# TalShor/SciLMM

Measured on AMD Instinct MI355X. Metric: REML factorize+solve nnz(L)/s (simulated pedigree, fp64), higher is better.
Workload: dtype f64

## Files before the change

scilmm_amd/csrc/dev.h:

```cpp
#pragma once
#include <hip/hip_runtime.h>

#include <algorithm>
#include <cstdlib>
#include <optional>
#include <string>
#include <type_traits>
#include <vector>

#include "../../include/scilmm_hip.h"
#include "plan_types.h"
#include "handles.h"

namespace scilmm {

struct Tuning {
  int reserve_cus = 0;
  int side_streams = 2;
  bool no_mfma = false;
  bool trsm_lite = true;
  std::optional<bool> dense;
  std::optional<bool> outside;
  bool outside_merge = true;
  std::optional<int> outside_chunks;
  bool outside_prio = false;
  std::optional<double> cell_limit;
  bool no_lookahead = false;
  int look_depth = 2;
  bool host_cells = false;
  bool no_splitk = false;
  int64_t target_items = 1024;
  int64_t min_item = 24;
  int64_t max_item = 96;
  std::optional<int64_t> dense_items;
  int64_t dense_fill = 256;
  std::optional<bool> dense_taper;
  std::optional<int> dist_group;
  bool dist_nosplit = false;
  int chain_cap = 2048;
  int chain_wide = 12;
  bool no_chain = false;
  int64_t push_slice = 512;
  bool shadow = true;
  int chain_wide_t = 256;
  int chain_full_t = 768;
  bool sinv_generic = false;
};

inline Tuning read_tuning() {
  Tuning t;
  const char* gate = getenv("SCILMM_TUNING");
  if (!(gate && gate[0] == '1')) return t;
  auto env = [](const char* name) { return getenv(name); };
  auto is1 = [&](const char* name) { const char* e = env(name); return e && e[0] == '1'; };
  auto not0 = [&](const char* name) { const char* e = env(name); return !(e && e[0] == '0'); };
  const char* e;
  if ((e = env("SCILMM_RESERVE_CUS"))) t.reserve_cus = atoi(e);
  if ((e = env("SCILMM_SIDE_STREAMS"))) t.side_streams = atoi(e);
  t.no_mfma = is1("SCILMM_NO_MFMA");
  t.trsm_lite = not0("SCILMM_TRSM_LITE");
  if ((e = env("SCILMM_DENSE"))) t.dense = e[0] != '0';
  if ((e = env("SCILMM_OUTSIDE"))) t.outside = e[0] != '0';
  t.outside_merge = not0("SCILMM_OUTSIDE_MERGE");
  if ((e = env("SCILMM_OUTSIDE_CHUNKS"))) t.outside_chunks = atoi(e);
  t.outside_prio = is1("SCILMM_OUTSIDE_PRIO");
  if ((e = env("SCILMM_CELL_LIMIT"))) t.cell_limit = atof(e);
  t.no_lookahead = is1("SCILMM_NO_LOOKAHEAD");
  if ((e = env("SCILMM_LOOK_DEPTH"))) t.look_depth = std::max(1, atoi(e));
  t.host_cells = is1("SCILMM_HOST_CELLS");
  t.no_splitk = is1("SCILMM_NO_SPLITK");
  if ((e = env("SCILMM_TARGET_ITEMS"))) t.target_items = atoll(e);
  if ((e = env("SCILMM_MIN_ITEM"))) t.min_item = atoll(e);
  if ((e = env("SCILMM_MAX_ITEM"))) t.max_item = atoll(e);
  if ((e = env("SCILMM_DENSE_ITEMS"))) t.dense_items = atoll(e);
  if ((e = env("SCILMM_DENSE_FILL"))) t.dense_fill = atoll(e);
  if ((e = env("SCILMM_DENSE_TAPER"))) t.dense_taper = e[0] == '1';
  if ((e = env("SCILMM_DIST_GROUP"))) t.dist_group = atoi(e);
  t.dist_nosplit = is1("SCILMM_DIST_NOSPLIT");
  if ((e = env("SCILMM_CHAIN_CAP"))) t.chain_cap = atoi(e);
  if ((e = env("SCILMM_CHAIN_WIDE"))) t.chain_wide = atoi(e);
  t.no_chain = is1("SCILMM_NO_CHAIN");
  if ((e = env("SCILMM_PUSH_SLICE"))) t.push_slice = atoll(e);
  t.shadow = not0("SCILMM_SHADOW");
  if ((e = env("SCILMM_CHAIN_WIDE_T"))) t.chain_wide_t = atoi(e);
  if ((e = env("SCILMM_CHAIN_FULL_T"))) t.chain_full_t = atoi(e);
  t.sinv_generic = is1("SCILMM_SINV_GENERIC");
  return t;
}

inline bool verbose() { return getenv("SCILMM_VERBOSE") != nullptr; }

struct Dev {
  int device = 0;
  hipStream_t stream = nullptr;
  Tuning tune;
  int prio_lo = 0, prio_hi = 0;
  DevSym v{};
  std::vector<void*> allocs;
  int32_t* d_level_tiles = nullptr;
  int32_t* d_level_fronts = nullptr;
  int32_t* d_level_pairs = nullptr;
  int32_t* d_all_fronts = nullptr;
  std::vector<double*> vals;
  std::vector<uint8_t> have_vals;
  double* W = nullptr;
  double* X = nullptr;
  double* IO = nullptr;
  size_t io_cap = 0;
  double* partial = nullptr;
  int64_t nwaves_quad = 0;
  double* d_out = nullptr;
  bool use_mfma = true;
  bool trsm_lite = true;
  hipEvent_t ev[8];
  scilmm_timing timing{};
  bool quad_pending = false;
  bool attrs_set = false;
  ComboDesc* d_combos = nullptr;
// ... 49 lines not shown
  std::vector<hipEvent_t> batch_ev;
  std::vector<hipEvent_t> bpev;
  std::vector<int32_t> last_own_level;
  hipStream_t bstream = nullptr;
  hipStream_t comm = nullptr;
  std::vector<hipEvent_t> done_ev;
  double* ACC = nullptr;
  int32_t* d_col_front = nullptr;
  int64_t* d_yoff = nullptr;
  double* d_ybuf = nullptr;
  int32_t* d_sinv_pre_tiles = nullptr;
  std::vector<int64_t> sinv_pre_ptr;
  std::vector<int32_t> sinv_tail_front;
  int32_t* d_sinv_tail_fronts = nullptr;
  SinvWork* d_sinv_work = nullptr;
  std::vector<int64_t> sinv_work_ptr;
  bool work_external = false;
  bool outside_on = false;
  int32_t tail_level = 0;
  std::vector<uint8_t> outside_desc;
  OutsideWork* d_owork = nullptr;
  int32_t* d_grp_next = nullptr;
  int32_t* d_grp_t0 = nullptr;
  int64_t n_owork = 0;
  int32_t* d_tail_front = nullptr;
  uint8_t* d_keep_front = nullptr;
  hipStream_t outside_st = nullptr;
  std::vector<int64_t> ochunk_ptr;
  std::vector<hipEvent_t> out_evs;
  std::vector<int32_t> out_wait_chunk;
  bool dense_on = false;
  int front_bits = 64;
  double* d_zeros = nullptr;
  DenseWork* d_dwork_e = nullptr;
  DenseWork* d_dwork_l = nullptr;
  std::vector<int64_t> dwork_e_ptr, dwork_l_ptr;
  std::vector<int64_t> dwork_l_mid;
  int64_t n_late_split = 0;
  int look_depth = 2;
  int rhs_pending = -1;
  int32_t chain_T = 0, chain_l0 = 0;
  int32_t* d_chain = nullptr;
  int32_t* d_colmap = nullptr;
  int32_t* d_cf_ptr = nullptr;
  ChainPair* d_cf = nullptr;
  int32_t* d_cb_ptr = nullptr;
  ChainPair* d_cb = nullptr;
  int64_t* d_cg_ptr = nullptr;
  int32_t* d_cg_pairs = nullptr;
  int64_t chain_groups = 0;
  int32_t* d_cg_slot = nullptr;
  int32_t* d_fold = nullptr;
  int64_t n_fold = 0;
  double* d_push_partial = nullptr;
  int32_t* d_chain_flags = nullptr;
  int32_t* d_chain_err = nullptr;
  int32_t* h_chain_err = nullptr;
  int32_t chain_epoch = 0;
  std::vector<hipEvent_t> pev;
  bool det = false;
  PullPlan pull{};
  int32_t* d_pull_level_segs = nullptr;
  int32_t* d_pull_fold = nullptr;
  double* d_pull_partial = nullptr;
  uint8_t* d_chain_mask = nullptr;
  const int64_t* d_pat_rowptr = nullptr;
// ... 57 lines not shown
```

scilmm_amd/csrc/engine.hip:

```cpp
#include <hip/hip_runtime.h>

#include <algorithm>
#include <atomic>
#include <chrono>
#include <functional>
#include <thread>
#include <cmath>
#include <cstdio>
#include <cstdlib>
#include <cstring>
#include <string>
#include <vector>

#include "../../include/scilmm_hip.h"
#include <hipcub/hipcub.hpp>

#include "kernels.hip.h"
#include "dev.h"
#include "host_threads.h"

using namespace scilmm;

namespace {

// ... 105 lines not shown
  int32_t tail_front(int32_t l) const { return dist ? D->tail_of_level[l] : -1; }
  bool has_early(int32_t l) const {
    return D->early_ptr[l + 1] > D->early_ptr[l] || D->cellset[0].level_ptr[l + 1] > D->cellset[0].level_ptr[l] ||
           D->dwork_e_ptr[l + 1] > D->dwork_e_ptr[l];
  }
  bool deferred(int32_t le) const { return D->outside_on && le >= D->tail_level; }
  int mark(int32_t l, ProfEvent e, hipStream_t stream) {
    if (prof) HIPCHK(hipEventRecord(D->pev[(size_t)PEV_PER_LEVEL * l + e], stream));
    return SCILMM_OK;
  }

  int prepare_shadow() {
    const bool want = D->front_bits == 32 && D->dense_on && read_tuning().shadow;
    if (want && !fac->L32) {
      fac->base32 = S.sn_loff[S.dense_first];
      const size_t cnt32 = (size_t)(D->nL_local - fac->base32) + 16384;
      if (hipMalloc((void**)&fac->L32, sizeof(float) * cnt32) != hipSuccess) {
        (void)hipGetLastError();
        fac->L32 = nullptr;
      } else {
        HIPCHK(hipMemsetAsync(fac->L32, 0, sizeof(float) * cnt32, st));
      }
    } else if (!want && fac->L32) {
      HIPCHK(hipStreamSynchronize(st));
      (void)hipFree(fac->L32);
      fac->L32 = nullptr;
    }
    return SCILMM_OK;
  }

  int assemble(const double* sigma2) {
    HIPCHK(hipEventRecord(D->ev[0], st));
    HIPCHK(hipMemsetAsync(fac->L, 0, sizeof(double) * (size_t)std::max<int64_t>(D->nL_local, 1), st));
    int32_t big = 0x7fffffff;
    HIPCHK(hipMemcpyAsync(fac->status, &big, sizeof(int32_t), hipMemcpyHostToDevice, st));
    ValPtrs gen{}, dia{};
    for (int k = 0; k < S.K; ++k) {
      ValPtrs& t = S.is_diag[k] ? dia : gen;
      if (t.count >= 8) {
        sym->err = "more than 8 matrices of one kind";
        return SCILMM_ERR_ARG;
      }
      t.v[t.count] = D->vals[k];
      t.s2[t.count] = sigma2[k];
      t.count++;
    }
    if (S.nnz_pattern > 0) {
      int blocks = (int)std::min<int64_t>((S.nnz_pattern + 255) / 256, 256 * 16);
      hipLaunchKernelGGL(k_assemble, dim3(blocks), dim3(256), 0, st, S.nnz_pattern, D->v.asm_dst, gen, fac->L);
      launches++;
    }
    if (dia.count > 0 && S.n > 0) {
      hipLaunchKernelGGL(k_add_diag, dim3((S.n + 255) / 256), dim3(256), 0, st, S.n, D->v.diag_dst, dia, fac->L);
      launches++;
    }
    HIPCHK(hipEventRecord(D->ev[1], st));
    HIPCHK(hipEventRecord(D->ev_asm, st));
    HIPCHK(hipStreamWaitEvent(D->side, D->ev_asm, 0));
    HIPCHK(hipStreamWaitEvent(D->side2, D->ev_asm, 0));
    if (D->side3) HIPCHK(hipStreamWaitEvent(D->side3, D->ev_asm, 0));
    if (D->outside_st) HIPCHK(hipStreamWaitEvent(D->outside_st, D->ev_asm, 0));
    if (dist) {
      HIPCHK(hipStreamWaitEvent(D->bstream, D->ev_asm, 0));
      HIPCHK(hipStreamWaitEvent(D->comm, D->ev_asm, 0));
    }
    return SCILMM_OK;
  }

  int prepare_profiling() {
    D->n_late_split = 0;
    if (prof && D->pev.size() < (size_t)PEV_PER_LEVEL * S.nlevels) {
      size_t old = D->pev.size();
      D->pev.resize((size_t)PEV_PER_LEVEL * S.nlevels, nullptr);
      for (size_t i = old; i < D->pev.size(); ++i) HIPCHK(hipEventCreate(&D->pev[i]));
    }
    if (prof && dist && D->bpev.size() < 2 * D->batch_ev.size()) {
      size_t old = D->bpev.size();
      D->bpev.resize(2 * D->batch_ev.size(), nullptr);
      for (size_t i = old; i < D->bpev.size(); ++i) HIPCHK(hipEventCreate(&D->bpev[i]));
    }
    return SCILMM_OK;
  }

  int early(int32_t l) {
    const int64_t e0 = D->early_ptr[l], e1 = D->early_ptr[l + 1];
    if (!has_early(l)) return SCILMM_OK;
    const int sidx = D->serial_early ? 0 : l % D->nside;
    hipStream_t sd = sidx == 0 ? D->side : (sidx == 1 ? D->side2 : D->side3);
    double* scratch = D->scratch + (size_t)sidx * half;
    if (l >= D->look_depth + 1) HIPCHK(hipStreamWaitEvent(sd, D->lev_ev[2 * (l - D->look_depth - 1)], 0));
    if (D->outside_on && l >= D->tail_level && D->out_wait_chunk[(size_t)l] >= 0)
      HIPCHK(hipStreamWaitEvent(sd, D->out_evs[(size_t)D->out_wait_chunk[(size_t)l]], 0));
    TRY(mark(l, PEV_EARLY_BEGIN, sd));
    update(sd, D->d_work_early + e0, e1 - e0, scratch);
    TRY(mark(l, PEV_DENSE_E_BEGIN, sd));
    dense(sd, D->d_dwork_e + D->dwork_e_ptr[l], D->dwork_e_ptr[l + 1] - D->dwork_e_ptr[l], scratch);
    TRY(mark(l, PEV_DENSE_E_END, sd));
    TRY(mark(l, PEV_EARLY_END, sd));
    reduce(sd, D->d_red_tiles_e + D->red_ptr_e[l], D->red_ptr_e[l + 1] - D->red_ptr_e[l], D->d_tile_pslot_e, D->d_tile_pnseg_e, scratch);
    TRY(cells(sd, 0, l));
    HIPCHK(hipEventRecord(D->lev_ev[2 * l + 1], sd));
    return SCILMM_OK;
  }

  int late_updates(int32_t l) {
    double* sh = late_scratch();
    if (D->outside_on && l >= D->tail_level && D->out_wait_chunk[(size_t)l] >= 0 &&
        (l == D->tail_level || D->out_wait_chunk[(size_t)l] != D->out_wait_chunk[(size_t)l - 1]))
      HIPCHK(hipStreamWaitEvent(st, D->out_evs[(size_t)D->out_wait_chunk[(size_t)l]], 0));
    const int32_t tf = tail_front(l), Wg = D->dist_Wg;
    const int32_t jj = tf >= 0 ? tf - D->dist_first : -1, grp = tf >= 0 ? jj / Wg : -1;
    const bool own_tail = tf >= 0 && D->keep_front[tf];
    const bool split_late = own_tail && D->dwork_l_mid[(size_t)l] < D->dwork_l_ptr[l + 1];
    if (has_early(l)) HIPCHK(hipStreamWaitEvent(st, D->lev_ev[2 * l + 1], 0));
    if (own_tail) {
      if (grp >= 2) HIPCHK(hipStreamWaitEvent(st, D->batch_ev[grp - 2], 0));
      const int32_t q_end = split_late ? jj - 1 : jj;
      for (int32_t q = std::max(0, (grp - 1) * Wg); q < q_end; ++q) HIPCHK(hipStreamWaitEvent(st, D->lev_ev[2 * S.sn_level[D->dist_first + q]], 0));
    }
    TRY(mark(l, PEV_LATE_BEGIN, st));
    update(st, D->d_work + D->work_ptr[l], D->work_ptr[l + 1] - D->work_ptr[l], sh);
    TRY(mark(l, PEV_DENSE_L_BEGIN, st));
    dense(st, D->d_dwork_l + D->dwork_l_ptr[l], (split_late ? D->dwork_l_mid[(size_t)l] : D->dwork_l_ptr[l + 1]) - D->dwork_l_ptr[l], sh);
    TRY(mark(l, PEV_DENSE_L_END, st));
    if (split_late) {
      HIPCHK(hipStreamWaitEvent(st, D->lev_ev[2 * S.sn_level[D->dist_first + jj - 1]], 0));
      TRY(mark(l, PEV_DENSE_N_BEGIN, st));
      dense(st, D->d_dwork_l + D->dwork_l_mid[(size_t)l], D->dwork_l_ptr[l + 1] - D->dwork_l_mid[(size_t)l], sh);
      TRY(mark(l, PEV_DENSE_N_END, st));
      D->n_late_split++;
    }
    return mark(l, PEV_LATE_END, st);
  }

  int factor_panel(int32_t l) {
    const int64_t t0 = D->lv_tile_ptr[l], t1 = D->lv_tile_ptr[l + 1];
    const int32_t f0 = D->lv_ptr[l], f1 = D->lv_ptr[l + 1];
    const double* sh = late_scratch();
    TRY(cells(st, 1, l));
    TRY(mark(l, PEV_CELLS_END, st));
    if (f1 > f0) {
      const size_t sm_potrf = sizeof(double) * (size_t)((NB / 2) * (NB + 1) + NJB * 16 * 17 + 32);
      hipLaunchKernelGGL(k_potrf, dim3((unsigned)(f1 - f0)), dim3(256), sm_potrf, st, D->v, D->d_level_fronts + f0, fac->L,
                         fac->invD, fac->logd, fac->status, (const int32_t*)D->d_tile_pslot, (const int32_t*)D->d_tile_pnseg, sh);
      launches++;
    }
    TRY(mark(l, PEV_POTRF_END, st));
    trsm(st, D->d_level_tiles + t0, t1 - t0, sh);
    if (fac->L32) {
      for (int32_t q = f0; q < f1; ++q) {
        const int32_t fr = D->lv_fronts[(size_t)q];
        if (fr < S.dense_first || !D->keep_front[fr]) continue;
        shadow(st, fr, S.sn_loff[fr + 1] - S.sn_loff[fr]);
      }
    }
    return mark(l, PEV_LEVEL_END, st);
  }

  void shadow(hipStream_t stream, int32_t fr, int64_t cnt) {
    hipLaunchKernelGGL(k_shadow, dim3((unsigned)std::min<int64_t>((cnt + 255) / 256, 8192)), dim3(256), 0, stream,
                       (const double*)(fac->L + D->loff[fr]), fac->L32 + (D->loff[fr] - fac->base32), cnt);
// ... 6 lines not shown
    HIPCHK(hipEventRecord(D->done_ev[l], st));
    HIPCHK(hipStreamWaitEvent(D->comm, D->done_ev[l], 0));
    if (!D->keep_front[tf]) {
      const int32_t gd = (jj - D->dist_G) / D->dist_Wg;
      if (jj >= D->dist_G) {
        HIPCHK(hipStreamWaitEvent(D->comm, D->batch_ev[gd], 0));
        for (int32_t q = std::min<int32_t>(gd + 1, (int32_t)D->last_own_level.size() - 1); q >= 0; --q)
          if (D->last_own_level[q] >= 0) {
            HIPCHK(hipStreamWaitEvent(D->comm, D->done_ev[D->last_own_level[q]], 0));
            break;
          }
      }
    }
    const int64_t pm = S.sn_rowptr[tf + 1] - S.sn_rowptr[tf], pw = S.sn_start[tf + 1] - S.sn_start[tf];
    int rcm = sym->comm_fn(sym->comm_ctx, 0, 0, D->loff[tf], pm * pw, root);
    if (rcm == 0) rcm = sym->comm_fn(sym->comm_ctx, 0, 1, S.inv_off[tf], pw * pw, root);
    if (rcm == 0) rcm = sym->comm_fn(sym->comm_ctx, 0, 2, tf, 1, root);
    if (rcm != 0) {
      sym->err = "multi-GPU: the communication callback failed";
      return SCILMM_ERR_DEVICE;
    }
    if (fac->L32 && !D->keep_front[tf]) shadow(D->comm, tf, pm * pw);
    HIPCHK(hipEventRecord(D->lev_ev[2 * l], D->comm));
    last_tail_level = l;
    return SCILMM_OK;
  }

  int batch(int32_t grp) {
    hipStream_t bs = D->bstream;
    const int32_t q_end = std::min((grp + 1) * D->dist_Wg, S.nsuper - D->dist_first);
    for (int32_t q = grp * D->dist_Wg; q < q_end; ++q) HIPCHK(hipStreamWaitEvent(bs, D->lev_ev[2 * S.sn_level[D->dist_first + q]], 0));
    if (D->outside_on) HIPCHK(hipStreamWaitEvent(bs, D->out_evs.back(), 0));
    if (prof) HIPCHK(hipEventRecord(D->bpev[2 * (size_t)grp], bs));
    dense(bs, D->d_dwork_b + D->dbatch_ptr[grp], D->dbatch_ptr[grp + 1] - D->dbatch_ptr[grp], nullptr);
    if (prof) HIPCHK(hipEventRecord(D->bpev[2 * (size_t)grp + 1], bs));
    HIPCHK(hipEventRecord(D->batch_ev[grp], bs));
    return SCILMM_OK;
  }

  int outside_and_deferred_early(int32_t l) {
    HIPCHK(hipStreamWaitEvent(D->outside_st, D->lev_ev[2 * l], 0));
    for (size_t og = 0; og + 1 < D->ochunk_ptr.size(); ++og) {
      outside(D->outside_st, (const OutsideWork*)D->d_owork + D->ochunk_ptr[og], D->ochunk_ptr[og + 1] - D->ochunk_ptr[og]);
      HIPCHK(hipGetLastError());
      HIPCHK(hipEventRecord(D->out_evs[og], D->outside_st));
    }
    for (int32_t le = std::max(D->tail_level, 1); le <= l + D->look_depth && le < S.nlevels; ++le) TRY(early(le));
    return SCILMM_OK;
  }

  int exchange_status() {
    if (last_tail_level >= 0) HIPCHK(hipStreamWaitEvent(st, D->lev_ev[2 * last_tail_level], 0));
    if (!D->batch_ev.empty()) HIPCHK(hipStreamWaitEvent(st, D->batch_ev.back(), 0));
    hipLaunchKernelGGL(k_status_pack, dim3(1), dim3(1), 0, st, (const int32_t*)fac->status, fac->logd + S.nsuper);
    HIPCHK(hipEventRecord(D->ev_x0, st));
    HIPCHK(hipStreamWaitEvent(D->comm, D->ev_x0, 0));
    if (sym->comm_fn(sym->comm_ctx, 2, 2, S.nsuper, 1, 0) != 0) {
      sym->err = "multi-GPU: the communication callback failed";
      return SCILMM_ERR_DEVICE;
    }
    HIPCHK(hipEventRecord(D->ev_x1, D->comm));
    HIPCHK(hipStreamWaitEvent(st, D->ev_x1, 0));
    hipLaunchKernelGGL(k_status_unpack, dim3(1), dim3(1), 0, st, (const double*)(fac->logd + S.nsuper), fac->status);
    return SCILMM_OK;
  }
};

// ... 1221 lines not shown
```

scilmm_amd/csrc/kernels.hip.h:

```cpp
#pragma once
#include <hip/hip_runtime.h>
#ifndef SCILMM_UPD_WAVES
#define SCILMM_UPD_WAVES 2
#endif
#include <stdint.h>

#include "plan_types.h"

namespace scilmm {

typedef double d4 __attribute__((ext_vector_type(4)));

constexpr int NJB = NB / 16;
constexpr int KCS = 16;
constexpr int LDA = TM + 16;
constexpr int LDB = NB + 16;
constexpr int LDP = 34;

__device__ __forceinline__ d4 mfma_f64(double a, double b, d4 c) {
  return __builtin_amdgcn_mfma_f64_16x16x4f64(a, b, c, 0, 0, 0);
}

__global__ void k_assemble(int64_t nnz, const int64_t* __restrict__ dst, ValPtrs vp, double* __restrict__ L) {
  int64_t stride = (int64_t)gridDim.x * blockDim.x;
// ... 310 lines not shown
  }
}


#ifndef SCILMM_DENSE_ABL
#define SCILMM_DENSE_ABL 0
#endif
#ifndef SCILMM_DENSE_VEC
#define SCILMM_DENSE_VEC 1
#endif
constexpr int DTR = 2 * TM;
constexpr int KBA = 64;
constexpr int LDA2 = DTR + 16;

#ifdef SCILMM_DENSE_CLK
__device__ unsigned long long g_dense_clk[2];
#endif

__device__ __forceinline__ int64_t uniform_i64(int64_t x) {
  const uint64_t v = (uint64_t)x;
  const uint32_t lo = __builtin_amdgcn_readfirstlane((uint32_t)v), hi = __builtin_amdgcn_readfirstlane((uint32_t)(v >> 32));
  return (int64_t)(((uint64_t)hi << 32) | lo);
}
__device__ __forceinline__ double ld_off(const double* base, uint32_t voff8) {
  return *(const double*)((const char*)base + voff8);
}
__device__ __forceinline__ int uniform_int(int v) { return __builtin_amdgcn_readfirstlane(v); }
typedef __attribute__((address_space(3))) void* lds_vptr;
typedef const __attribute__((address_space(1))) void* gl_vptr;

#ifndef SCILMM_DENSE_B_SG
#define SCILMM_DENSE_B_SG 1
#endif
__global__ __launch_bounds__(512, 1) void k_dense_b(DevSym S, int32_t dense_first, const DenseWork* __restrict__ work,
                                                    double* __restrict__ L, double* __restrict__ scratch,
                                                    const double* __restrict__ zeros) {
  static_assert(NB == 128 && DTR == 256, "k_dense_b: 8 waves x 32 rows, one B k-row per DMA instruction");
  extern __shared__ __attribute__((aligned(16))) double smem[];
  const int tid = threadIdx.x, lane = tid & 63, wv = __builtin_amdgcn_readfirstlane(tid >> 6);
  const int li = lane & 15, lk = lane >> 4;
  const DenseWork wk = work[blockIdx.x];
  const int32_t j = wk.front;
  const int32_t c0j = S.sn_start[j], wj = S.sn_start[j + 1] - c0j;
  const int32_t mj = S.n - c0j;
  const int32_t R0 = wk.ti0 * TM;
  const int32_t nrow = min(wk.ntiles * TM, mj - R0);
  const int32_t ia = 32 * wv + li, ib_ = ia + 16;
  const int32_t ra0 = R0 + (ia < nrow ? ia : 0);
  const int32_t ra1 = R0 + (ib_ < nrow ? ib_ : 0);
  const int32_t b_off = 2 * lane < wj ? 2 * lane : 0;
  const double* zsrc = zeros + 2 * lane;
  struct Chunk { const double* Pd; int32_t md; int kc; uint32_t v0, v1; };
  int32_t kd = wk.k0, kk0 = 0;
  int32_t d_wd = 0, d_md = 0;
  const double* d_P0 = nullptr;
  auto next_chunk = [&]() {
    if (kk0 == 0) {
      const int32_t d = dense_first + kd;
      const int32_t c0d = S.sn_start[d];
      d_wd = __builtin_amdgcn_readfirstlane(S.sn_start[d + 1] - c0d);
      d_md = __builtin_amdgcn_readfirstlane(S.n - c0d);
      d_P0 = L + uniform_i64(S.sn_loff[d] + (c0j - c0d));
    }
    Chunk c;
    c.md = d_md;
    c.Pd = d_P0 + (int64_t)kk0 * d_md;
    c.kc = min(KBA, d_wd - kk0);
    c.v0 = (uint32_t)(lk * c.md + ra0) * 8u;
    c.v1 = (uint32_t)(lk * c.md + ra1) * 8u;
    kk0 += KBA;
    if (kk0 >= d_wd) { kk0 = 0; ++kd; }
    return c;
  };
  auto issue_B = [&](const Chunk& c, int b) {
    double* Bs = smem + b * KBA * LDB;
    if (c.kc == KBA) {
      const double* p = c.Pd + (int64_t)wv * c.md + b_off;
      const int64_t step = 8 * (int64_t)c.md;
#pragma unroll
      for (int i = 0; i < KBA / 8; ++i)
        __builtin_amdgcn_global_load_lds((gl_vptr)(p + i * step), (lds_vptr)(Bs + (wv + 8 * i) * LDB), 16, 0, 0);
      return;
    }
#pragma unroll
    for (int i = 0; i < KBA / 8; ++i) {
      const int kr = wv + 8 * i;
      __builtin_amdgcn_global_load_lds((gl_vptr)(kr < c.kc ? c.Pd + (int64_t)kr * c.md + b_off : zsrc), (lds_vptr)(Bs + kr * LDB), 16, 0, 0);
    }
  };
  auto load_A = [&](const Chunk& c, int s, double (&ra)[4][2]) {
    const int klast = (c.kc - 1) & ~3;
#pragma unroll
    for (int q = 0; q < 4; ++q) {
      const double* sp = c.Pd + (int64_t)min(16 * s + 4 * q, klast) * c.md;
      ra[q][0] = ld_off(sp, c.v0);
      ra[q][1] = ld_off(sp, c.v1);
    }
  };
  d4 acc16[NJB][2];
#pragma unroll
  for (int a = 0; a < NJB; ++a) { acc16[a][0] = (d4){0.0, 0.0, 0.0, 0.0}; acc16[a][1] = (d4){0.0, 0.0, 0.0, 0.0}; }
  if (wk.k0 >= wk.k1) return;
  double rA[2][4][2];
  double bf[2][NJB];
  auto ldB = [&](const double* Bc, int k4, double (&b)[NJB]) {
#pragma unroll
    for (int jb = 0; jb < NJB; ++jb) b[jb] = Bc[(k4 + lk) * LDB + 16 * jb + li];
  };
  auto mma = [&](const double (&b)[NJB], double a0, double a1) {
#pragma unroll
    for (int jb = 0; jb < NJB; ++jb) {
      acc16[jb][0] = mfma_f64(b[jb], a0, acc16[jb][0]);
      acc16[jb][1] = mfma_f64(b[jb], a1, acc16[jb][1]);
    }
  };
  Chunk cur = next_chunk();
  issue_B(cur, 0);
  load_A(cur, 0, rA[0]);
  bool more = kd < wk.k1;
  Chunk nxt = cur;
  if (more) {
    nxt = next_chunk();
    issue_B(nxt, 1);
  }
  asm volatile("s_waitcnt vmcnt(0)" ::: "memory");
  __syncthreads();
  int buf = 0;
  ldB(smem, 0, bf[0]);
  while (true) {
    const double* Bc = smem + buf * KBA * LDB;
    const double* Bn = smem + (buf ^ 1) * KBA * LDB;
    bool more2 = false;
    Chunk nn = nxt;
#pragma unroll
    for (int t = 0; t < 16; ++t) {
      const int s = t >> 2, q = t & 3;
      if (q == 0) {
        if (s < 3) load_A(cur, s + 1, rA[(s + 1) & 1]);
        else if (more) load_A(nxt, 0, rA[0]);
      }
      if (t < 15) {
        ldB(Bc, 4 * (t + 1), bf[(t + 1) & 1]);
      } else if (more) {
        asm volatile("s_waitcnt vmcnt(0) lgkmcnt(0)" ::: "memory");
        __builtin_amdgcn_s_barrier();
        ldB(Bn, 0, bf[0]);
        more2 = kd < wk.k1;
        if (more2) {
          nn = next_chunk();
          issue_B(nn, buf);
        }
      }
      mma(bf[t & 1], rA[s & 1][q][0], rA[s & 1][q][1]);
#if SCILMM_DENSE_B_SG
      if (t < 15) {
#pragma unroll
        for (int g = 0; g < 4; ++g) {
          __builtin_amdgcn_sched_group_barrier(0x100, 1, 0);
          __builtin_amdgcn_sched_group_barrier(0x008, 4, 0);
        }
      }
#endif
      __builtin_amdgcn_sched_barrier(0);
    }
    if (!more) break;
    cur = nxt;
    nxt = nn;
    more = more2;
    buf ^= 1;
  }
  double* P = L + S.sn_loff[j];
#pragma unroll
  for (int jb = 0; jb < NJB; ++jb)
#pragma unroll
    for (int ib = 0; ib < 2; ++ib)
#pragma unroll
      for (int r = 0; r < 4; ++r) {
        const int i = ib == 0 ? ia : ib_, jc = 16 * jb + lk + 4 * r;
        const double v = acc16[jb][ib][r];
        const int h = i >> 7;
        const int32_t slot = h ? wk.slot1 : wk.slot0;
        if (slot < 0) {
          if (i < nrow && jc < wj) P[(int64_t)jc * mj + R0 + i] -= v;
        } else if (h < wk.ntiles) {
          scratch[(int64_t)slot * (TM * NB) + jc * TM + (i & (TM - 1))] = v;
        }
      }
}

typedef float f4 __attribute__((ext_vector_type(4)));
constexpr int LDA2F = DTR + 16;
constexpr int LDBF = NB + 16;

__global__ __launch_bounds__(512, 1) void k_dense32(DevSym S, int32_t dense_first, const DenseWork* __restrict__ work,
                                                    double* __restrict__ L, double* __restrict__ scratch) {
  extern __shared__ __attribute__((aligned(16))) double smem[];
  float* Abuf = (float*)smem;
  float* Bbuf = Abuf + 2 * KC * LDA2F;
  const int tid = threadIdx.x, lane = tid & 63, wv = tid >> 6;
  const DenseWork wk = work[blockIdx.x];
  const int32_t j = wk.front;
  const int32_t c0j = S.sn_start[j], wj = S.sn_start[j + 1] - c0j;
  const int32_t mj = S.n - c0j;
  const int32_t R0 = wk.ti0 * TM;
  const int32_t nrow = min(wk.ntiles * TM, mj - R0);
  typedef double d2 __attribute__((ext_vector_type(2)));
  typedef float f2 __attribute__((ext_vector_type(2)));
  constexpr int NPA = KC / 4, NPB = KC / 8;
  const int pa = tid & (DTR / 2 - 1), ka = tid >> 7;
  const int pb = tid & (NB / 2 - 1), kb = tid >> 6;
  const int ra_row = 2 * pa < nrow ? 2 * pa : 0, rb_col = 2 * pb < wj ? 2 * pb : 0;
  d2 ra[NPA], rb[NPB];
  int32_t kd = wk.k0, kk0 = 0;
  int kc_ld = 0;
  auto load_chunk = [&]() {
    const int32_t d = dense_first + kd;
    const int32_t c0d = S.sn_start[d], wd = S.sn_start[d + 1] - c0d;
    const int64_t md = S.n - c0d;
    const double* Pd = L + S.sn_loff[d] + (int64_t)kk0 * md + (c0j - c0d);
    kc_ld = min(KC, wd - kk0);
// ... 2273 lines not shown
```

scilmm_amd/csrc/launch.hip.h:

```cpp
#pragma once

namespace {

inline int64_t max_groups(unsigned threads) { return (int64_t)(((uint64_t)1 << 32) / threads) - 1; }

struct FactorLaunch {
  Dev* const D;
  scilmm_factor* const fac;
  int64_t launches = 0;

  void update(hipStream_t stream, const UpdWork* work, int64_t cnt, double* scratch_half) {
#ifdef SCILMM_DIAG
    if (D->ablate == 4) return;
#endif
    const size_t sm_upd = sizeof(double) * (size_t)(2 * KC * LDA + 2 * KC * LDB) + sizeof(int32_t) * TM;
    const auto k = D->use_mfma ? k_update2<true> : k_update2<false>;
    for (int64_t o = 0; o < cnt; o += max_groups(UPD_THREADS)) {
      const unsigned c = (unsigned)std::min<int64_t>(cnt - o, max_groups(UPD_THREADS));
      hipLaunchKernelGGL(k, dim3(c), dim3(UPD_THREADS), sm_upd, stream, D->v, work + o, D->d_combos, fac->L, scratch_half);
      launches++;
    }
  }

  void dense(hipStream_t stream, const DenseWork* dw, int64_t cnt, double* scratch_half) {
    const int32_t dense_first = fac->sym->S->dense_first;
    for (int64_t o = 0; o < cnt; o += max_groups(1024)) {
      const unsigned c = (unsigned)std::min<int64_t>(cnt - o, max_groups(1024));
      if (D->front_bits == 32 && fac->L32)
        hipLaunchKernelGGL(k_dense_h, dim3(2 * c), dim3(512), dense_h_lds, stream, D->v, dense_first, dw + o, fac->L, (const float*)fac->L32,
                           fac->base32, scratch_half, (const float*)D->d_zeros);
      else if (D->front_bits == 32)
        hipLaunchKernelGGL(k_dense32, dim3(c), dim3(512), sizeof(float) * (size_t)(2 * KC * LDA2F + 2 * KC * LDBF), stream, D->v,
                           dense_first, dw + o, fac->L, scratch_half);
      else
        hipLaunchKernelGGL(k_dense_b, dim3(c), dim3(512), sizeof(double) * (size_t)(2 * KBA * LDB), stream, D->v, dense_first, dw + o,
                           fac->L, scratch_half, (const double*)D->d_zeros);
      launches++;
    }
  }

  void reduce(hipStream_t stream, const int32_t* tiles, int64_t cnt, const int32_t* pslot, const int32_t* pnseg, const double* slabs) {
    const int64_t per = max_groups(128) / (NB / 4);
    for (int64_t o = 0; o < cnt; o += per) {
      const int64_t c = std::min(cnt - o, per);
      hipLaunchKernelGGL(k_reduce, dim3((unsigned)((NB / 4) * c)), dim3(128), 0, stream, D->v, tiles + o, pslot, pnseg, slabs, fac->L);
      launches++;
    }
  }

  int cells(hipStream_t stream, int which, int32_t l) {
    const Dev::CellSet& CS = D->cellset[which];
    const int64_t u0 = CS.level_ptr[l], u1 = CS.level_ptr[l + 1];
    if (u1 <= u0) return SCILMM_OK;
#ifdef SCILMM_DIAG
    if (D->ablate == 5) return SCILMM_OK;
#endif
    const int64_t nshort = CS.level_short[l], nlong = (u1 - u0) - nshort;
    const int64_t nblk = (nshort + 255) / 256 + (nlong + 3) / 4;
    if (nblk > max_groups(256)) {
      fac->sym->err = "cell plan: one level has more target cells than a dispatch can hold";
      return SCILMM_ERR_ARG;
    }
    hipLaunchKernelGGL(k_sparse_cells, dim3((unsigned)nblk), dim3(256), 0, stream, u0, nshort, u1 - u0, (const int64_t*)CS.dst,
                       (const int64_t*)CS.grp, (const int64_t*)CS.srct, (const int64_t*)CS.srcq, (const int32_t*)CS.md,
                       (const int32_t*)CS.wd, fac->L);
    launches++;
    return SCILMM_OK;
  }

// ... 96 lines not shown
```

scilmm_amd/csrc/plan.hip:

```cpp
#include <hip/hip_runtime.h>

#include <algorithm>
#include <atomic>
#include <chrono>
#include <functional>
#include <thread>
#include <cmath>
#include <cstdio>
#include <cstdlib>
#include <cstring>
#include <string>
#include <vector>

#include "dev.h"
#include "cellplan.hip.h"
#include "host_threads.h"

namespace scilmm {

void dev_free(void* p) {
  Dev* D = (Dev*)p;
  if (!D) return;
  for (void* a : D->allocs) (void)hipFree(a);
  for (double* v : D->vals)
// ... 536 lines not shown
    for (auto& e : D->out_evs) HIPCHK(hipEventCreateWithFlags(&e, hipEventDisableTiming));
    if ((st = upload(sym, D, ow, &D->d_owork)) != SCILMM_OK) return st;
    {
      if ((st = upload(sym, D, grp_next, &D->d_grp_next)) != SCILMM_OK) return st;
      if ((st = upload(sym, D, grp_t0, &D->d_grp_t0)) != SCILMM_OK) return st;
    }
    if ((st = upload(sym, D, tf, &D->d_tail_front)) != SCILMM_OK) return st;
    if ((st = upload(sym, D, D->keep_front, &D->d_keep_front)) != SCILMM_OK) return st;
    {
      HIPCHK(hipStreamCreateWithPriority(&D->outside_st, hipStreamNonBlocking, D->tune.outside_prio ? D->prio_hi : D->prio_lo));
    }
    if (pb.verbose) {
      fprintf(stderr, "[scilmm plan] k_outside: %lld block-pair items of prelude fronts below level %d (tail starts at column %d), %d chunks by first panel:",
              (long long)D->n_owork, D->tail_level, c0_tail, nch);
      for (int32_t g = 0; g < nch; ++g) fprintf(stderr, " [%d..: %lld]", chunk_lo[g] - S.dense_first, (long long)(D->ochunk_ptr[g + 1] - D->ochunk_ptr[g]));
      fprintf(stderr, "\n");
    }
  }
  return SCILMM_OK;
}

int upload_symbolic(scilmm_symbolic* sym, Dev* D) {
  const Symbolic& S = *sym->S;
  const std::vector<int64_t>& LOFF = D->loff;
  D->v.n = S.n;
  D->v.nsuper = S.nsuper;
  int st;
#define UP(field, vec)                                          \
  if ((st = upload(sym, D, S.vec, &D->v.field)) != SCILMM_OK) return st;
  UP(sn_start, sn_start)
  UP(sn_rowptr, sn_rowptr)
  UP(sn_rows, sn_rows)
  if ((st = upload(sym, D, D->loff, &D->v.sn_loff)) != SCILMM_OK) return st;
  UP(inv_off, inv_off)
  UP(upd_src, upd_src)
  UP(upd_p0, upd_p0)
  UP(upd_p1, upd_p1)
  UP(tile_front, tile_front)
  UP(tile_base, tile_base)
  if (distributed_tail(D, S)) {
    std::vector<int64_t> ad(S.asm_dst.size()), dd(S.diag_dst.size());
    const int nth = std::max(1, std::min(16, scilmm::host_threads()));
    std::vector<std::thread> pool;
    auto part = [&](int q) {
      for (int32_t f = q; f < S.nsuper; f += nth) {
        const bool keep = D->keep_front[f] != 0;
        const int64_t delta = LOFF[f] - S.sn_loff[f];
        for (int32_t j = S.sn_start[f]; j < S.sn_start[f + 1]; ++j) {
          dd[(size_t)j] = keep ? S.diag_dst[(size_t)j] + delta : -1;
          for (int64_t e = S.pat_colptr[j]; e < S.pat_colptr[j + 1]; ++e) ad[(size_t)e] = keep ? S.asm_dst[(size_t)e] + delta : -1;
        }
      }
    };
    for (int q = 1; q < nth; ++q) pool.emplace_back(part, q);
    part(0);
    for (auto& th : pool) th.join();
    if ((st = upload(sym, D, ad, &D->v.asm_dst)) != SCILMM_OK) return st;
    if ((st = upload(sym, D, dd, &D->v.diag_dst)) != SCILMM_OK) return st;
  } else {
    UP(asm_dst, asm_dst)
    UP(diag_dst, diag_dst)
  }
  UP(pat_colptr, pat_colptr)
  UP(pat_row, pat_row)
  UP(perm, perm)
#undef UP
// ... 694 lines not shown
    }
    max_slots = std::max(max_slots, slots);
    D->lev_cost_e.push_back(total_e);
    D->lev_cost_l.push_back(total_l);
    D->work_ptr[l + 1] = (int64_t)work.size();
    D->early_ptr[l + 1] = (int64_t)work_early.size();
    D->red_ptr[l + 1] = (int64_t)red_tiles.size();
    D->red_ptr_e[l + 1] = (int64_t)red_tiles_e.size();
  }

  int plan_dist_batches(scilmm_symbolic* sym) {
    int st;
    const int32_t nT = S.nsuper - S.dense_first;
    const int32_t ngroups = (nT + Wg - 1) / Wg;
    std::vector<DenseWork> dwork_b;
    D->dbatch_ptr.assign((size_t)ngroups + 1, 0);
    std::vector<std::pair<int32_t, int32_t>> runs;
    for (int32_t g = 0; g < ngroups; ++g) {
      for (int32_t jj = (g + 2) * Wg; jj < nT; ++jj) {
        const int32_t fr = S.dense_first + jj;
        if (!D->keep_front[fr]) continue;
        if (active_runs(jj, g * Wg, std::min((g + 1) * Wg, nT), runs) == 0) continue;
        const int32_t k0 = runs.front().first, k1 = runs.back().second;
        const int32_t ntl = (int32_t)(S.tile_base[fr + 1] - S.tile_base[fr]);
        const std::vector<uint8_t>& pon = own_pair_on[(size_t)jj];
        for (int32_t q = 0; q < ntl; q += 2) {
          if (!pon.empty() && !pon[(size_t)(q / 2)]) continue;
          dwork_b.push_back(DenseWork{fr, q, std::min<int32_t>(2, ntl - q), k0, k1, -1, -1, 0});
        }
      }
      D->dbatch_ptr[(size_t)g + 1] = (int64_t)dwork_b.size();
    }
    if (dwork_b.empty()) dwork_b.push_back(DenseWork{});
    if ((st = upload(sym, D, dwork_b, &D->d_dwork_b)) != SCILMM_OK) return st;
    if (pb.verbose)
      fprintf(stderr, "[scilmm plan] rank %d: %lld batch items in %d source groups of %d tail panels\n", D->rank,
              (long long)D->dbatch_ptr[(size_t)ngroups], ngroups, Wg);
    return SCILMM_OK;
  }

  int upload_items(scilmm_symbolic* sym) {
    int st;
    {
      if (dwork_e.empty()) dwork_e.push_back(DenseWork{});
      if (dwork_l.empty()) dwork_l.push_back(DenseWork{});
      if ((st = upload(sym, D, dwork_e, &D->d_dwork_e)) != SCILMM_OK) return st;
      if ((st = upload(sym, D, dwork_l, &D->d_dwork_l)) != SCILMM_OK) return st;
      if (pb.verbose && dense_pairs_all > 0)
        fprintf(stderr, "[scilmm plan] dense tail: %lld of %lld (target, descendant) panel pairs carry true entries, %lld of %lld target tile pairs are reached by a descendant (the others are padding only and skipped)\n",
                (long long)dense_pairs_kept, (long long)dense_pairs_all, (long long)dense_tiles_kept, (long long)dense_tiles_all);
      if (pb.verbose)
        fprintf(stderr, "[scilmm plan] dense tail: fronts %d..%d (%d wide), %lld early + %lld late implicit items (k_dense_b)\n",
                S.dense_first, S.nsuper - 1, tail_w,
                (long long)D->dwork_e_ptr[S.nlevels], (long long)D->dwork_l_ptr[S.nlevels]);
    }
    if (work_early.empty()) work_early.push_back(UpdWork{0, -1, 0, 0});
    if ((st = upload(sym, D, work_early, &D->d_work_early)) != SCILMM_OK) return st;
    if (red_tiles_e.empty()) red_tiles_e.push_back(0);
    if ((st = upload(sym, D, red_tiles_e, &D->d_red_tiles_e)) != SCILMM_OK) return st;
    if ((st = upload(sym, D, pslot_e, &D->d_tile_pslot_e)) != SCILMM_OK) return st;
    if ((st = upload(sym, D, pnseg_e, &D->d_tile_pnseg_e)) != SCILMM_OK) return st;
    if (red_tiles.empty()) red_tiles.push_back(0);
    if ((st = upload(sym, D, red_tiles, &D->d_red_tiles)) != SCILMM_OK) return st;
    if (work.empty()) work.push_back(UpdWork{0, -1, 0, 0});
    if ((st = upload(sym, D, work, &D->d_work)) != SCILMM_OK) return st;
    if ((st = upload(sym, D, pslot, &D->d_tile_pslot)) != SCILMM_OK) return st;
    if ((st = upload(sym, D, pnseg, &D->d_tile_pnseg)) != SCILMM_OK) return st;
    void* sc = nullptr;
    HIPCHK(hipMalloc(&sc, sizeof(double) * (size_t)4 * (size_t)D->max_slots * TM * NB));
    D->allocs.push_back(sc);
    D->scratch = (double*)sc;
    return SCILMM_OK;
  }
};

int cut_work_items(scilmm_symbolic* sym, Dev* D, PlanBuild& pb) {
  WorkCut wc(*sym->S, D, pb);
  for (int32_t l = 0; l < sym->S->nlevels; ++l) wc.cut_level(l);
// ... 304 lines not shown
```

scilmm_amd/csrc/plan_types.h:

```cpp
#pragma once
#include <stdint.h>
#ifndef SCILMM_KC
#define SCILMM_KC 16
#endif
#ifndef SCILMM_NB
#define SCILMM_NB 128
#endif
#ifndef SCILMM_CW
#define SCILMM_CW 32
#endif

namespace scilmm {

constexpr int NB = SCILMM_NB;
constexpr int TM = 128;
constexpr int KC = SCILMM_KC;
constexpr int RPMAX = 128;
constexpr int CW = SCILMM_CW;

struct DevSym {
  int32_t n, nsuper;
  const int32_t* sn_start;
  const int64_t* sn_rowptr;
  const int32_t* sn_rows;
// ... 12 lines not shown
};

struct ValPtrs {
  const double* v[8];
  double s2[8];
  int32_t count;
};

struct ComboDesc {
  int64_t loff;
  int64_t rowoff;
  int32_t md, wd;
  int32_t ta, nt;
  int32_t p0, nq;
  int32_t ip0;
  int32_t jp0;
  int32_t ilo, ihi;
  int32_t jlo, jhi;
};

struct UpdWork {
  int32_t tile;
  int32_t slot;
  int64_t cb, ce;
};

struct DenseWork {
  int32_t front;
  int32_t ti0;
  int32_t ntiles;
  int32_t k0, k1;
  int32_t slot0, slot1;
  int32_t pad;
};

struct OutsideWork {
  int32_t d;
  int32_t t0;
  int32_t bi, bj;
};

struct CellSrc { int64_t st, sq; int32_t md, wd; };

struct PullPlan {
  const int32_t* seg_front;
  const int64_t* seg_ptr;
  const int32_t* seg_slot;
  const int32_t* front_seg;
};

struct ChainPair {
  int32_t other;
  int32_t p0, nq;
  int32_t jp0;
  int32_t map;
};

struct SinvOwner {
  int64_t loff;
  const int32_t* rows;
  int32_t c0, m;
  int32_t tail;
};

struct SinvWork {
  int32_t front;
  int32_t q;
// ... 5 lines not shown
```

Baseline: 1.426 billion.

## Chain dense tail items per workgroup via atomic tickets with precomputed front table

The dense tail kernel now lets each workgroup pull several work items from a global atomic ticket counter, up to a chunk budget, instead of handling exactly one item per block. It writes back accumulators at each item boundary and keeps the double-buffered pipeline running across items. Per-item constants (front start, width, height, L offset, chunk count) are precomputed on the host into a widened 64-byte DenseWork, and a packed per-front table replaces the scattered sn_start/sn_loff lookups. The aim is to cut pipeline refill and launch imbalance on short items, at the cost of extra barriers and atomics per item, a per-factorization ticket memset, and a larger work record.

Measured after the change: 1.422 billion. Within noise of the previous version (-0.3%).

```diff
diff --git a/scilmm_amd/csrc/dev.h b/scilmm_amd/csrc/dev.h
--- a/scilmm_amd/csrc/dev.h
+++ b/scilmm_amd/csrc/dev.h
@@ -44,6 +44,7 @@
   bool shadow = true;
   int chain_wide_t = 256;
   int chain_full_t = 768;
+  std::optional<int> dense_chain;
   bool sinv_generic = false;
 };
 
@@ -84,6 +85,7 @@
   t.shadow = not0("SCILMM_SHADOW");
   if ((e = env("SCILMM_CHAIN_WIDE_T"))) t.chain_wide_t = atoi(e);
   if ((e = env("SCILMM_CHAIN_FULL_T"))) t.chain_full_t = atoi(e);
+  if ((e = env("SCILMM_DENSE_CHAIN"))) t.dense_chain = std::max(0, atoi(e));
   t.sinv_generic = is1("SCILMM_SINV_GENERIC");
   return t;
 }
@@ -199,6 +201,11 @@
   bool dense_on = false;
   int front_bits = 64;
   double* d_zeros = nullptr;
+  TailFront* d_tail_tab = nullptr;
+  int32_t* d_tickets = nullptr;
+  int64_t n_tickets = 0;
+  std::vector<int32_t> dlong_e, dlong_l, dlong_n;
+  std::vector<int32_t> dlong_b;
   DenseWork* d_dwork_e = nullptr;
   DenseWork* d_dwork_l = nullptr;
   std::vector<int64_t> dwork_e_ptr, dwork_l_ptr;
diff --git a/scilmm_amd/csrc/engine.hip b/scilmm_amd/csrc/engine.hip
--- a/scilmm_amd/csrc/engine.hip
+++ b/scilmm_amd/csrc/engine.hip
@@ -161,6 +161,7 @@
   int assemble(const double* sigma2) {
     HIPCHK(hipEventRecord(D->ev[0], st));
     HIPCHK(hipMemsetAsync(fac->L, 0, sizeof(double) * (size_t)std::max<int64_t>(D->nL_local, 1), st));
+    if (D->d_tickets) HIPCHK(hipMemsetAsync(D->d_tickets, 0, sizeof(int32_t) * (size_t)D->n_tickets, st));
     int32_t big = 0x7fffffff;
     HIPCHK(hipMemcpyAsync(fac->status, &big, sizeof(int32_t), hipMemcpyHostToDevice, st));
     ValPtrs gen{}, dia{};
@@ -223,7 +224,7 @@
     TRY(mark(l, PEV_EARLY_BEGIN, sd));
     update(sd, D->d_work_early + e0, e1 - e0, scratch);
     TRY(mark(l, PEV_DENSE_E_BEGIN, sd));
-    dense(sd, D->d_dwork_e + D->dwork_e_ptr[l], D->dwork_e_ptr[l + 1] - D->dwork_e_ptr[l], scratch);
+    dense(sd, D->d_dwork_e + D->dwork_e_ptr[l], D->dwork_e_ptr[l + 1] - D->dwork_e_ptr[l], scratch, l, D->dlong_e[(size_t)l]);
     TRY(mark(l, PEV_DENSE_E_END, sd));
     TRY(mark(l, PEV_EARLY_END, sd));
     reduce(sd, D->d_red_tiles_e + D->red_ptr_e[l], D->red_ptr_e[l + 1] - D->red_ptr_e[l], D->d_tile_pslot_e, D->d_tile_pnseg_e, scratch);
@@ -250,12 +251,14 @@
     TRY(mark(l, PEV_LATE_BEGIN, st));
     update(st, D->d_work + D->work_ptr[l], D->work_ptr[l + 1] - D->work_ptr[l], sh);
     TRY(mark(l, PEV_DENSE_L_BEGIN, st));
-    dense(st, D->d_dwork_l + D->dwork_l_ptr[l], (split_late ? D->dwork_l_mid[(size_t)l] : D->dwork_l_ptr[l + 1]) - D->dwork_l_ptr[l], sh);
+    dense(st, D->d_dwork_l + D->dwork_l_ptr[l], (split_late ? D->dwork_l_mid[(size_t)l] : D->dwork_l_ptr[l + 1]) - D->dwork_l_ptr[l], sh,
+          S.nlevels + l, split_late ? D->dlong_l[(size_t)l] : std::max(D->dlong_l[(size_t)l], D->dlong_n[(size_t)l]));
     TRY(mark(l, PEV_DENSE_L_END, st));
     if (split_late) {
       HIPCHK(hipStreamWaitEvent(st, D->lev_ev[2 * S.sn_level[D->dist_first + jj - 1]], 0));
       TRY(mark(l, PEV_DENSE_N_BEGIN, st));
-      dense(st, D->d_dwork_l + D->dwork_l_mid[(size_t)l], D->dwork_l_ptr[l + 1] - D->dwork_l_mid[(size_t)l], sh);
+      dense(st, D->d_dwork_l + D->dwork_l_mid[(size_t)l], D->dwork_l_ptr[l + 1] - D->dwork_l_mid[(size_t)l], sh, 2 * (int64_t)S.nlevels + l,
+            D->dlong_n[(size_t)l]);
       TRY(mark(l, PEV_DENSE_N_END, st));
       D->n_late_split++;
     }
@@ -328,7 +331,8 @@
     for (int32_t q = grp * D->dist_Wg; q < q_end; ++q) HIPCHK(hipStreamWaitEvent(bs, D->lev_ev[2 * S.sn_level[D->dist_first + q]], 0));
     if (D->outside_on) HIPCHK(hipStreamWaitEvent(bs, D->out_evs.back(), 0));
     if (prof) HIPCHK(hipEventRecord(D->bpev[2 * (size_t)grp], bs));
-    dense(bs, D->d_dwork_b + D->dbatch_ptr[grp], D->dbatch_ptr[grp + 1] - D->dbatch_ptr[grp], nullptr);
+    dense(bs, D->d_dwork_b + D->dbatch_ptr[grp], D->dbatch_ptr[grp + 1] - D->dbatch_ptr[grp], nullptr, 3 * (int64_t)S.nlevels + grp,
+          D->dlong_b[(size_t)grp]);
     if (prof) HIPCHK(hipEventRecord(D->bpev[2 * (size_t)grp + 1], bs));
     HIPCHK(hipEventRecord(D->batch_ev[grp], bs));
     return SCILMM_OK;
diff --git a/scilmm_amd/csrc/kernels.hip.h b/scilmm_amd/csrc/kernels.hip.h
--- a/scilmm_amd/csrc/kernels.hip.h
+++ b/scilmm_amd/csrc/kernels.hip.h
@@ -366,44 +366,87 @@
 #ifndef SCILMM_DENSE_B_SG
 #define SCILMM_DENSE_B_SG 1
 #endif
-__global__ __launch_bounds__(512, 1) void k_dense_b(DevSym S, int32_t dense_first, const DenseWork* __restrict__ work,
+constexpr size_t dense_b_lds = sizeof(double) * (size_t)(2 * KBA * LDB);
+__global__ __launch_bounds__(512, 1) void k_dense_b(int32_t n, const TailFront* __restrict__ tf, const DenseWork* __restrict__ work,
+                                                    int32_t cnt, int32_t* __restrict__ ticket, int32_t budget,
                                                     double* __restrict__ L, double* __restrict__ scratch,
                                                     const double* __restrict__ zeros) {
   static_assert(NB == 128 && DTR == 256, "k_dense_b: 8 waves x 32 rows, one B k-row per DMA instruction");
   extern __shared__ __attribute__((aligned(16))) double smem[];
+  __shared__ int32_t tk_lds;
   const int tid = threadIdx.x, lane = tid & 63, wv = __builtin_amdgcn_readfirstlane(tid >> 6);
   const int li = lane & 15, lk = lane >> 4;
-  const DenseWork wk = work[blockIdx.x];
-  const int32_t j = wk.front;
-  const int32_t c0j = S.sn_start[j], wj = S.sn_start[j + 1] - c0j;
-  const int32_t mj = S.n - c0j;
-  const int32_t R0 = wk.ti0 * TM;
-  const int32_t nrow = min(wk.ntiles * TM, mj - R0);
   const int32_t ia = 32 * wv + li, ib_ = ia + 16;
-  const int32_t ra0 = R0 + (ia < nrow ? ia : 0);
-  const int32_t ra1 = R0 + (ib_ < nrow ? ib_ : 0);
-  const int32_t b_off = 2 * lane < wj ? 2 * lane : 0;
   const double* zsrc = zeros + 2 * lane;
-  struct Chunk { const double* Pd; int32_t md; int kc; uint32_t v0, v1; };
-  int32_t kd = wk.k0, kk0 = 0;
+  struct Chunk { const double* Pd; int32_t md; int kc; uint32_t v0, v1; int32_t item, last; };
+  int32_t g_item = 0, g_kd = 0, g_k1 = 0, g_kk0 = 0, g_c0j = 0;
+  int32_t ra0 = 0, ra1 = 0, b_off = 0;
+  bool g_open = true;
+  int32_t taken = 0;
+  typedef int32_t tf4 __attribute__((ext_vector_type(4)));
+  auto fetch_tf = [&](int32_t k) {
+    uint64_t a = (uint64_t)(tf + k);
+    asm volatile("" : "+v"(a));
+    return *(const __attribute__((address_space(1))) tf4*)a;
+  };
+  tf4 nx = {0, 0, 0, 0};
   int32_t d_wd = 0, d_md = 0;
   const double* d_P0 = nullptr;
+  auto begin_item = [&](int32_t idx) {
+    const DenseWork w = work[idx];
+    if (w.k0 >= w.k1) return false;
+    g_item = idx;
+    g_kd = w.k0;
+    g_k1 = w.k1;
+    g_kk0 = 0;
+    g_c0j = w.c0j;
+    const int32_t R0 = w.ti0 * TM;
+    const int32_t nrow = min(w.ntiles * TM, w.mj - R0);
+    ra0 = R0 + (ia < nrow ? ia : 0);
+    ra1 = R0 + (ib_ < nrow ? ib_ : 0);
+    b_off = 2 * lane < w.wj ? 2 * lane : 0;
+    nx = fetch_tf(w.k0);
+    taken += w.nchunks;
+    return true;
+  };
+  auto have_more = [&]() {
+    if (g_kd < g_k1) return true;
+    if (!g_open) return false;
+    g_open = false;
+    int32_t idx;
+    if (ticket == nullptr) {
+      if (taken > 0) return false;
+      idx = blockIdx.x;
+    } else {
+      if (taken > 0 && taken >= budget) return false;
+      __syncthreads();
+      if (tid == 0) tk_lds = atomicAdd(ticket, 1);
+      __syncthreads();
+      idx = __builtin_amdgcn_readfirstlane(tk_lds);
+      if (idx >= cnt) return false;
+    }
+    g_open = begin_item(idx);
+    return g_open;
+  };
   auto next_chunk = [&]() {
-    if (kk0 == 0) {
-      const int32_t d = dense_first + kd;
-      const int32_t c0d = S.sn_start[d];
-      d_wd = __builtin_amdgcn_readfirstlane(S.sn_start[d + 1] - c0d);
-      d_md = __builtin_amdgcn_readfirstlane(S.n - c0d);
-      d_P0 = L + uniform_i64(S.sn_loff[d] + (c0j - c0d));
+    if (g_kk0 == 0) {
+      const int32_t c0d = __builtin_amdgcn_readfirstlane(nx.z);
+      d_wd = __builtin_amdgcn_readfirstlane(nx.w);
+      d_md = n - c0d;
+      const int64_t lo = (int64_t)(((uint64_t)(uint32_t)__builtin_amdgcn_readfirstlane(nx.y) << 32) | (uint32_t)__builtin_amdgcn_readfirstlane(nx.x));
+      d_P0 = L + (lo + (g_c0j - c0d));
+      nx = fetch_tf(min(g_kd + 1, g_k1 - 1));
     }
     Chunk c;
     c.md = d_md;
-    c.Pd = d_P0 + (int64_t)kk0 * d_md;
-    c.kc = min(KBA, d_wd - kk0);
+    c.Pd = d_P0 + (int64_t)g_kk0 * d_md;
+    c.kc = min(KBA, d_wd - g_kk0);
     c.v0 = (uint32_t)(lk * c.md + ra0) * 8u;
     c.v1 = (uint32_t)(lk * c.md + ra1) * 8u;
-    kk0 += KBA;
-    if (kk0 >= d_wd) { kk0 = 0; ++kd; }
+    g_kk0 += KBA;
+    if (g_kk0 >= d_wd) { g_kk0 = 0; ++g_kd; }
+    c.item = g_item;
+    c.last = g_kd >= g_k1 ? 1 : 0;
     return c;
   };
   auto issue_B = [&](const Chunk& c, int b) {
@@ -434,7 +477,7 @@
   d4 acc16[NJB][2];
 #pragma unroll
   for (int a = 0; a < NJB; ++a) { acc16[a][0] = (d4){0.0, 0.0, 0.0, 0.0}; acc16[a][1] = (d4){0.0, 0.0, 0.0, 0.0}; }
-  if (wk.k0 >= wk.k1) return;
+  if (!have_more()) return;
   double rA[2][4][2];
   double bf[2][NJB];
   auto ldB = [&](const double* Bc, int k4, double (&b)[NJB]) {
@@ -451,7 +494,7 @@
   Chunk cur = next_chunk();
   issue_B(cur, 0);
   load_A(cur, 0, rA[0]);
-  bool more = kd < wk.k1;
+  bool more = have_more();
   Chunk nxt = cur;
   if (more) {
     nxt = next_chunk();
@@ -466,6 +509,7 @@
     const double* Bn = smem + (buf ^ 1) * KBA * LDB;
     bool more2 = false;
     Chunk nn = nxt;
+    const DenseWork ew = work[cur.last ? cur.item : 0];
 #pragma unroll
     for (int t = 0; t < 16; ++t) {
       const int s = t >> 2, q = t & 3;
@@ -479,7 +523,7 @@
         asm volatile("s_waitcnt vmcnt(0) lgkmcnt(0)" ::: "memory");
         __builtin_amdgcn_s_barrier();
         ldB(Bn, 0, bf[0]);
-        more2 = kd < wk.k1;
+        more2 = have_more();
         if (more2) {
           nn = next_chunk();
           issue_B(nn, buf);
@@ -497,29 +541,37 @@
 #endif
       __builtin_amdgcn_sched_barrier(0);
     }
-    if (!more) break;
+    if (cur.last) {
+      const int32_t R0 = ew.ti0 * TM, mj = ew.mj, wj = ew.wj;
+      const int32_t nrow = min(ew.ntiles * TM, mj - R0);
+      double* P = L + ew.loff;
+      int32_t ia_e = ia, lk_e = lk;
+      asm volatile("" : "+v"(ia_e), "+v"(lk_e));
+#pragma unroll
+      for (int jb = 0; jb < NJB; ++jb)
+#pragma unroll
+        for (int ib = 0; ib < 2; ++ib)
+#pragma unroll
+          for (int r = 0; r < 4; ++r) {
+            const int i = ib == 0 ? ia_e : ia_e + 16, jc = 16 * jb + lk_e + 4 * r;
+            const double v = acc16[jb][ib][r];
+            const int h = i >> 7;
+            const int32_t slot = h ? ew.slot1 : ew.slot0;
+            if (slot < 0) {
+              if (i < nrow && jc < wj) P[(int64_t)jc * mj + R0 + i] -= v;
+            } else if (h < ew.ntiles) {
+              scratch[(int64_t)slot * (TM * NB) + jc * TM + (i & (TM - 1))] = v;
+            }
+          }
+      if (!more) break;
+#pragma unroll
+      for (int a = 0; a < NJB; ++a) { acc16[a][0] = (d4){0.0, 0.0, 0.0, 0.0}; acc16[a][1] = (d4){0.0, 0.0, 0.0, 0.0}; }
+    }
     cur = nxt;
     nxt = nn;
     more = more2;
     buf ^= 1;
   }
-  double* P = L + S.sn_loff[j];
-#pragma unroll
-  for (int jb = 0; jb < NJB; ++jb)
-#pragma unroll
-    for (int ib = 0; ib < 2; ++ib)
-#pragma unroll
-      for (int r = 0; r < 4; ++r) {
-        const int i = ib == 0 ? ia : ib_, jc = 16 * jb + lk + 4 * r;
-        const double v = acc16[jb][ib][r];
-        const int h = i >> 7;
-        const int32_t slot = h ? wk.slot1 : wk.slot0;
-        if (slot < 0) {
-          if (i < nrow && jc < wj) P[(int64_t)jc * mj + R0 + i] -= v;
-        } else if (h < wk.ntiles) {
-          scratch[(int64_t)slot * (TM * NB) + jc * TM + (i & (TM - 1))] = v;
-        }
-      }
 }
 
 typedef float f4 __attribute__((ext_vector_type(4)));
diff --git a/scilmm_amd/csrc/launch.hip.h b/scilmm_amd/csrc/launch.hip.h
--- a/scilmm_amd/csrc/launch.hip.h
+++ b/scilmm_amd/csrc/launch.hip.h
@@ -8,6 +8,7 @@
   Dev* const D;
   scilmm_factor* const fac;
   int64_t launches = 0;
+  std::optional<int> dense_chain = read_tuning().dense_chain;
 
   void update(hipStream_t stream, const UpdWork* work, int64_t cnt, double* scratch_half) {
 #ifdef SCILMM_DIAG
@@ -22,8 +23,9 @@
     }
   }
 
-  void dense(hipStream_t stream, const DenseWork* dw, int64_t cnt, double* scratch_half) {
+  void dense(hipStream_t stream, const DenseWork* dw, int64_t cnt, double* scratch_half, int64_t ticket, int32_t longest) {
     const int32_t dense_first = fac->sym->S->dense_first;
+    const int32_t budget = dense_chain.value_or(std::max(longest, 8));
     for (int64_t o = 0; o < cnt; o += max_groups(1024)) {
       const unsigned c = (unsigned)std::min<int64_t>(cnt - o, max_groups(1024));
       if (D->front_bits == 32 && fac->L32)
@@ -33,8 +35,8 @@
         hipLaunchKernelGGL(k_dense32, dim3(c), dim3(512), sizeof(float) * (size_t)(2 * KC * LDA2F + 2 * KC * LDBF), stream, D->v,
                            dense_first, dw + o, fac->L, scratch_half);
       else
-        hipLaunchKernelGGL(k_dense_b, dim3(c), dim3(512), sizeof(double) * (size_t)(2 * KBA * LDB), stream, D->v, dense_first, dw + o,
-                           fac->L, scratch_half, (const double*)D->d_zeros);
+        hipLaunchKernelGGL(k_dense_b, dim3(c), dim3(512), dense_b_lds, stream, D->v.n, (const TailFront*)D->d_tail_tab, dw + o, (int32_t)c,
+                           budget > 0 && o == 0 ? D->d_tickets + ticket : nullptr, budget, fac->L, scratch_half, (const double*)D->d_zeros);
       launches++;
     }
   }
diff --git a/scilmm_amd/csrc/plan.hip b/scilmm_amd/csrc/plan.hip
--- a/scilmm_amd/csrc/plan.hip
+++ b/scilmm_amd/csrc/plan.hip
@@ -592,6 +592,12 @@
   UP(sn_rowptr, sn_rowptr)
   UP(sn_rows, sn_rows)
   if ((st = upload(sym, D, D->loff, &D->v.sn_loff)) != SCILMM_OK) return st;
+  if (S.dense_first < S.nsuper) {
+    std::vector<TailFront> tab((size_t)(S.nsuper - S.dense_first));
+    for (int32_t f = S.dense_first; f < S.nsuper; ++f)
+      tab[(size_t)(f - S.dense_first)] = TailFront{D->loff[(size_t)f], S.sn_start[f], S.sn_start[f + 1] - S.sn_start[f]};
+    if ((st = upload(sym, D, tab, &D->d_tail_tab)) != SCILMM_OK) return st;
+  }
   UP(inv_off, inv_off)
   UP(upd_src, upd_src)
   UP(upd_p0, upd_p0)
@@ -1352,6 +1358,9 @@
       D->dbatch_ptr[(size_t)g + 1] = (int64_t)dwork_b.size();
     }
     if (dwork_b.empty()) dwork_b.push_back(DenseWork{});
+    fill_dense_consts(dwork_b.data(), (int64_t)dwork_b.size(), S.sn_start.data(), D->loff.data(), S.n, S.dense_first);
+    D->dlong_b.assign((size_t)ngroups, 0);
+    for (int32_t g = 0; g < ngroups; ++g) D->dlong_b[(size_t)g] = longest_item(dwork_b, D->dbatch_ptr[(size_t)g], D->dbatch_ptr[(size_t)g + 1]);
     if ((st = upload(sym, D, dwork_b, &D->d_dwork_b)) != SCILMM_OK) return st;
     if (pb.verbose)
       fprintf(stderr, "[scilmm plan] rank %d: %lld batch items in %d source groups of %d tail panels\n", D->rank,
@@ -1359,11 +1368,32 @@
     return SCILMM_OK;
   }
 
+  static int32_t longest_item(const std::vector<DenseWork>& w, int64_t a, int64_t b) {
+    int32_t m = 0;
+    for (int64_t i = a; i < b; ++i) m = std::max(m, w[(size_t)i].nchunks);
+    return m;
+  }
+
   int upload_items(scilmm_symbolic* sym) {
     int st;
     {
       if (dwork_e.empty()) dwork_e.push_back(DenseWork{});
       if (dwork_l.empty()) dwork_l.push_back(DenseWork{});
+      fill_dense_consts(dwork_e.data(), (int64_t)dwork_e.size(), S.sn_start.data(), D->loff.data(), S.n, S.dense_first);
+      fill_dense_consts(dwork_l.data(), (int64_t)dwork_l.size(), S.sn_start.data(), D->loff.data(), S.n, S.dense_first);
+      D->dlong_e.assign((size_t)std::max(S.nlevels, 1), 0);
+      D->dlong_l.assign((size_t)std::max(S.nlevels, 1), 0);
+      D->dlong_n.assign((size_t)std::max(S.nlevels, 1), 0);
+      for (int32_t l = 0; l < S.nlevels; ++l) {
+        D->dlong_e[(size_t)l] = longest_item(dwork_e, D->dwork_e_ptr[l], D->dwork_e_ptr[l + 1]);
+        D->dlong_l[(size_t)l] = longest_item(dwork_l, D->dwork_l_ptr[l], D->dwork_l_mid[(size_t)l]);
+        D->dlong_n[(size_t)l] = longest_item(dwork_l, D->dwork_l_mid[(size_t)l], D->dwork_l_ptr[l + 1]);
+      }
+      D->n_tickets = 3 * (int64_t)std::max(S.nlevels, 1) + (int64_t)D->dlong_b.size();
+      void* tk = nullptr;
+      HIPCHK(hipMalloc(&tk, sizeof(int32_t) * (size_t)D->n_tickets));
+      D->allocs.push_back(tk);
+      D->d_tickets = (int32_t*)tk;
       if ((st = upload(sym, D, dwork_e, &D->d_dwork_e)) != SCILMM_OK) return st;
       if ((st = upload(sym, D, dwork_l, &D->d_dwork_l)) != SCILMM_OK) return st;
       if (pb.verbose && dense_pairs_all > 0)
diff --git a/scilmm_amd/csrc/plan_types.h b/scilmm_amd/csrc/plan_types.h
--- a/scilmm_amd/csrc/plan_types.h
+++ b/scilmm_amd/csrc/plan_types.h
@@ -68,7 +68,30 @@
   int32_t k0, k1;
   int32_t slot0, slot1;
   int32_t pad;
+  int32_t c0j, wj, mj;
+  int32_t nchunks;
+  int64_t loff;
+  int64_t pad2;
 };
+static_assert(sizeof(DenseWork) == 64, "DenseWork: four 16-byte words");
+
+struct TailFront {
+  int64_t loff;
+  int32_t c0, w;
+};
+
+inline void fill_dense_consts(DenseWork* w, int64_t cnt, const int32_t* sn_start, const int64_t* loff, int32_t n, int32_t dense_first) {
+  for (int64_t i = 0; i < cnt; ++i) {
+    DenseWork& x = w[i];
+    if (x.k1 <= x.k0) continue;
+    x.c0j = sn_start[x.front];
+    x.wj = sn_start[x.front + 1] - x.c0j;
+    x.mj = n - x.c0j;
+    x.loff = loff[x.front];
+    x.nchunks = 0;
+    for (int32_t k = x.k0; k < x.k1; ++k) x.nchunks += (sn_start[dense_first + k + 1] - sn_start[dense_first + k] + 63) / 64;
+  }
+}
 
 struct OutsideWork {
   int32_t d;
```
